# sunzeyucmu/VAE-based-Music--Deep-Generative-Models

Measured on AMD Instinct MI355X. Metric: audio-samples/sec/GPU VQ-VAE train step, 44.1kHz 65536-frame chunks @1/2/4/8 GPU, higher is better.
Workload: dtype bf16; 1 GPU; SMALL_VQ_VAE 3-level VQ-VAE train step (BASELINE config 2); model=VQVAE levels=3 latent=64 K=2048 down_depth=[3,2,2] width=32 depth=4 dil=3, global_batch=32, seq_len=65536, parallelism=dp1, graph=True

## Files before the change

include/vqa.h:

```cpp
#ifndef VQA_H
#define VQA_H

#include <stddef.h>
#include <stdint.h>

#ifdef __cplusplus
extern "C" {
#endif

typedef void* vqa_stream_t;

enum { VQA_OK = 0, VQA_E_INVALID_ARG = -1, VQA_E_UNSUPPORTED = -2, VQA_E_HIP = -3 };
enum { VQA_F32 = 0, VQA_BF16 = 1 };

enum {
  VQA_PRE_RELU = 1,
  VQA_ADD_RESIDUAL = 2,
  VQA_POST_MASK = 4,
  VQA_X_F32 = 8,
  VQA_Y_F32 = 16
};

const char* vqa_get_last_error(void);
const char* vqa_version(void);
// ... 62 lines not shown
  VQA_ROUTE_CO1 = 0, VQA_ROUTE_CONV32 = 1, VQA_ROUTE_GATHER_MFMA = 2, VQA_ROUTE_CI1 = 3, VQA_ROUTE_THIN_O = 4,
  VQA_ROUTE_THIN = 5, VQA_ROUTE_DIRECT = 6, VQA_ROUTE_WGRAD_MFMA = 7, VQA_ROUTE_WGRAD_THIN = 8,
  VQA_ROUTE_WGRAD_DIRECT = 9, VQA_ROUTE_TWO_CALL = 10
};
#define VQA_ROUTE_DETAIL 8
int vqa_conv1d_route(int op, int B, int T_in, int T_out, int C_in, int C_out, int K, int stride, int dilation,
                     int pad_left, int flags, int dtype, int* detail);

int vqa_resblock_supported(int C, int dilation, int dtype);
int vqa_resblock_fwd(const void* x, const float* wa, const float* ba, const float* wb, const float* bb, void* y,
                     void* h_out, int B, int T, int C, int dilation, int dtype, vqa_stream_t stream);
int vqa_resblock_bwd(const void* dy, const void* x, const float* wa, const float* ba, const float* wb, const float* bb,
                     void* dx, float* dwa, float* dba, float* dwb, float* dbb, int B, int T, int C, int dilation,
                     int dtype, void* workspace, size_t ws_bytes, vqa_partials_desc* desc, vqa_stream_t stream);
size_t vqa_resblock_bwd_workspace(int B, int T, int C, int dilation, int dtype);

int vqa_dtail_supported(int C, int Cu, int K_up, int stride_up, int K_out, int C_out, int dtype);
size_t vqa_dtail_workspace(int B, int T, int C, int Cu, int dtype);
int vqa_dtail_fwd(const void* h, const float* w_up, const float* b_up, const float* w_out, const float* b_out,
                  float* y, int B, int T, int C, int Cu, int dtype, void* workspace, size_t ws_bytes,
                  vqa_stream_t stream);
int vqa_dtail_bwd(const float* dy, const void* h, const float* w_up, const float* b_up, const float* w_out,
                  const float* b_out, void* dh, float* dw_up, float* db_up, float* dw_out, float* db_out, int B,
                  int T, int C, int Cu, int dtype, void* workspace, size_t ws_bytes, vqa_stream_t stream);

int vqa_vq_sqnorm(const float* E, float* e_sqnorm, int D, int K, vqa_stream_t stream);
int vqa_vq_argmin(const void* z, const float* E, const float* e_sqnorm, int64_t* idx, float* min_dist,
                  int64_t N, int D, int K, int dtype, vqa_stream_t stream);
int vqa_vq_argmin_split(const void* z, const void* E3, const float* e_sqnorm, int64_t* idx, float* min_dist,
                        int64_t N, int D, int K, vqa_stream_t stream);
// ... 145 lines not shown
```

vae-based-music--deep-generative-models_amd/csrc/vqa_resblock.hip:

```cpp
#include "vqa_launch.h"
#include "vqa_mfma.h"
#include <algorithm>
#include <type_traits>

namespace vqa {

constexpr int RC = 32;
constexpr int RTM = 128;
constexpr int RMAXD = 32;

struct ResArgs {
  const void* x;
  const void* dy;
  void* y;
  void* h;
  const float* wa;
  const float* ba;
  const float* wb;
  const float* bb;
  float* part_a;
  float* part_b;
  int B, T, d;
  int ntm, ntiles, tpw, textra;
  int nwg;
};

template <class T> constexpr int rs_stride() { return RC + lds_pad<T>(); }
constexpr int round16(int v) { return (v + 15) & ~15; }
constexpr int kVmcnt0 = 0x0F70;

#ifdef VQA_RS_STAMPS
constexpr int kRsStampWgs = 1024;
__device__ unsigned long long g_rs_stamps[kRsStampWgs * 4 * 8];
#define RS_STAMP(i)                                                                                      \
  do {                                                                                                   \
    if (stamp_on && lane == 0 && blockIdx.x < kRsStampWgs)                                               \
      g_rs_stamps[(blockIdx.x * 4 + wave) * 8 + (i)] = __builtin_amdgcn_s_memtime();                     \
  } while (0)
#else
// ... 198 lines not shown

struct RsCursor {
  int n, tm;
  __device__ __forceinline__ void set(int tile, int ntm) {
    n = tile / ntm;
    tm = tile - n * ntm;
  }
  __device__ __forceinline__ void next(int ntm) {
    if (++tm == ntm) {
      tm = 0;
      ++n;
    }
  }
};

template <class T> constexpr int rs_pv() { return sizeof(T) == 2 ? 4 : 8; }

template <class T> constexpr int rs_ncc() { return RC / Mfma<T>::KS; }

template <class T, bool KPERM>
__device__ __forceinline__ void load_wfrags(typename Mfma<T>::frag (&wf)[3][2][rs_ncc<T>()], const float* w) {
  const int lane = threadIdx.x & 63, m = lane & 15, kc = rs_kcol<T, KPERM>(lane);
#pragma unroll
  for (int k = 0; k < 3; ++k)
#pragma unroll
    for (int mt = 0; mt < 2; ++mt)
#pragma unroll
      for (int s = 0; s < rs_ncc<T>(); ++s) {
        const int o = 8 * rs_sig(m >> 2) + 4 * mt + (m & 3);
        if constexpr (sizeof(T) == 2) {
// ... 69 lines not shown
  if constexpr (sizeof(T) == 2) {
    __builtin_amdgcn_sched_group_barrier(0x100, NJ * 3 * NCC + (ALDS ? 6 * NCC : 0), 0);
    __builtin_amdgcn_sched_group_barrier(0x008, NJ * 6 * NCC, 0);
  }
}

__device__ __forceinline__ f32x4 bias4(const float* b, int o) { return f32x4{b[o], b[o + 1], b[o + 2], b[o + 3]}; }

constexpr bool kRsFwdKperm = false;

template <class T> constexpr int rs_fwd_waves() { return sizeof(T) == 2 ? 3 : 2; }

constexpr int rs_fwd_rt(int dt) { return dt > 0 ? 176 : RTM; }
constexpr int rs_bwd_rt(int dt) { return (dt > 0 && dt <= 9) ? 160 : RTM; }

template <class T, int DT, int RT = rs_fwd_rt(DT)>
__global__ __launch_bounds__(256) __attribute__((amdgpu_waves_per_eu(rs_fwd_waves<T>(), 8)))
void resblock_fwd_kernel(ResArgs a) {
  constexpr int XS = rs_stride<T>(), HR = RT + 16, NT = RT / 16, NJ = (NT + 3) / 4;
  extern __shared__ __attribute__((aligned(16))) char smem[];
  T* X = (T*)smem;
  const int d = DT > 0 ? DT : a.d, XR = HR + 2 * d;
  T* H = X + XR * XS;
  const int wave = __builtin_amdgcn_readfirstlane(threadIdx.x >> 6), lane = threadIdx.x & 63;
  const int tbeg = blockIdx.x * a.tpw + min((int)blockIdx.x, a.textra),
            tend = tbeg + a.tpw + ((int)blockIdx.x < a.textra);
  if (tbeg >= tend) return;
  typename Mfma<T>::frag wfa[3][2][rs_ncc<T>()], wfb[3][2][rs_ncc<T>()];
  if constexpr (sizeof(T) == 2 && DT > 0) {
    bf16* img = (bf16*)(X + (HR + 2 * DT) * XS);
    f32x4 va[3 * RC * RC / 4 / 256], vb[3 * RC * RC / 4 / 256];
    load_w4(va, a.wa);
    load_w4(vb, a.wb);
// ... 2 lines not shown
    __syncthreads();
    frags_from_img<kRsFwdKperm>(wfa, img);
    frags_from_img<kRsFwdKperm>(wfb, img + kImgRows * kImgP);
  } else {
    load_wfrags<T, kRsFwdKperm>(wfa, a.wa);
    load_wfrags<T, kRsFwdKperm>(wfb, a.wb);
  }
  const int pn = rs_pi(lane & 15), oc = rs_ocol(lane);
  f32x4 bav[2], bbv[2];
#pragma unroll
  for (int mt = 0; mt < 2; ++mt) {
    bav[mt] = a.ba ? bias4(a.ba, oc + 4 * mt) : f32x4{0.f, 0.f, 0.f, 0.f};
    bbv[mt] = a.bb ? bias4(a.bb, oc + 4 * mt) : f32x4{0.f, 0.f, 0.f, 0.f};
  }
  const unsigned ibytes = (unsigned)a.T * RC * (unsigned)sizeof(T);
  auto load_x = [&](Rows32Buf<T, rs_pv<T>()>& bx, const RsCursor& c) {
    bx.load(rs_rsrc((const T*)a.x + (size_t)c.n * a.T * RC, ibytes), c.tm * RT - 1 - d);
  };
  Rows32Buf<T, rs_pv<T>()> nx;
  nx.init(XR, (XR + HR) * XS);
  RsCursor cur, ldc;
  cur.set(tbeg, a.ntm);
  ldc = cur;
  load_x(nx, ldc);
  nx.template store<false>(X);
  if (tbeg + 1 < tend) {
    ldc.next(a.ntm);
    load_x(nx, ldc);
  }
  __syncthreads();
  for (int tile = tbeg; tile < tend; ++tile, cur.next(a.ntm)) {
    const int n = cur.n, t0 = cur.tm * RT;
#ifdef VQA_RS_STAMPS
    const bool stamp_on = tile == tbeg + 4;
#endif
    RS_STAMP(0);
    const bool interior = t0 - 1 >= 0 && t0 - 1 + HR <= a.T;
    int ry[NJ];
    Raw8<T> xres[NJ];
#pragma unroll
// ... 28 lines not shown
          for (int mt = 0; mt < 2; ++mt) {
            v[mt] = acc[j][mt];
#pragma unroll
            for (int q = 0; q < 4; ++q) v[mt][q] = live ? fmaxf(v[mt][q], 0.f) : 0.f;
          }
          st8(H + i * XS + oc, v[0], v[1]);
          if (a.h && i >= 1 && i <= RT)
            st8_buf<T>(rs_rsrc((T*)a.h + (size_t)n * a.T * RC, ibytes), (r * RC + oc) * (int)sizeof(T), v[0], v[1]);
        }
      }
    }
    RS_STAMP(1);
    __syncthreads();
    RS_STAMP(2);
    if (tile + 1 < tend) {
      nx.template store<false>(X);
      if (tile + 2 < tend) {
        ldc.next(a.ntm);
        load_x(nx, ldc);
      }
    }
    RS_STAMP(3);
    {
      const __amdgpu_buffer_rsrc_t yr = rs_rsrc((T*)a.y + (size_t)n * a.T * RC, ibytes);
      f32x4 acc[NJ][2];
      conv_multi<T, false, kRsFwdKperm, false, NJ>(acc, wb_frag, H, ry, 1, bbv[0], bbv[1]);
#pragma unroll
      for (int j = 0; j < NJ; ++j) {
        if (wave + 4 * j >= NT) continue;
        const int tl = ry[j] + pn;
        f32x4 x0, x1;
        xres[j].unpack(x0, x1);
        st8_buf<T>(yr, ((t0 + tl) * RC + oc) * (int)sizeof(T), x0 + acc[j][0], x1 + acc[j][1]);
      }
    }
    RS_STAMP(4);
    if (tile + 1 < tend) __syncthreads();
    RS_STAMP(5);
  }
}

template <class T, int DT, int RT = rs_bwd_rt(DT), int HALVES = 1>
__global__ __launch_bounds__(256 * HALVES) void resblock_bwd_kernel(ResArgs a) {
  typedef Mfma<T> M;
  constexpr int NW = 4;
  constexpr int XS = rs_stride<T>(), NT = RT / 16;
  constexpr int NA = (NT + 1) / 2, NA1 = NA < 3 ? NA : 3, NA2 = NA - NA1;
  static_assert(NA2 >= 1 && NA2 <= 3, "dx: two batches per team-W wave");
  constexpr int DM = DT > 0 ? DT : RMAXD, HRM = round16(RT + 2 * DM);
  constexpr int NHT = HRM / 16, NP1 = (NHT + 3) / 4, P1A = NP1 < 3 ? NP1 : 3, P1B = NP1 - P1A;
  constexpr int NDH = (NHT + 1) / 2, DH1 = NDH < 3 ? NDH : 3, DH2 = NDH - DH1 < 3 ? NDH - DH1 : 3,
                DH3 = NDH - DH1 - DH2;
  static_assert(P1B <= 3 && DH3 <= 3, "recomputed rows: at most 24 16-row tiles");
  constexpr int PVX = ((HRM + 2 * DM) * RC * (int)sizeof(T) / 16 + 64 * NW - 1) / (64 * NW);
  constexpr int PVY = ((HRM + 2) * RC * (int)sizeof(T) / 16 + 64 * NW - 1) / (64 * NW);
  extern __shared__ __attribute__((aligned(16))) char smem[];
  const int d = DT > 0 ? DT : a.d, HR = round16(RT + 2 * d), XR = HR + 2 * d, YR = HR + 2;
  const int wave_g = __builtin_amdgcn_readfirstlane(threadIdx.x >> 6);
// ... 27 lines not shown
    frags_from_img<true>(wt, img + (team == 0 ? 1 : 2) * kImgRows * kImgP);
  } else {
    load_wfrags<T, true>(wfa, a.wa);
    load_wfrags_t<T>(wt, team == 0 ? a.wa : a.wb);
  }
  const int pn = rs_pi(lane & 15), oc = rs_ocol(lane);
  f32x4 bav[2];
#pragma unroll
  for (int mt = 0; mt < 2; ++mt) bav[mt] = a.ba ? bias4(a.ba, oc + 4 * mt) : f32x4{0.f, 0.f, 0.f, 0.f};
  f32x4 gw[2][3], gb = {0.f, 0.f, 0.f, 0.f};
#pragma unroll
  for (int o = 0; o < 2; ++o)
#pragma unroll
    for (int k = 0; k < 3; ++k) gw[o][k] = f32x4{0.f, 0.f, 0.f, 0.f};
  const int nht = HR / 16;

  const unsigned ibytes = (unsigned)a.T * RC * (unsigned)sizeof(T);
  auto load_tile = [&](Rows32Buf<T, PVX>& bx, Rows32Buf<T, PVY>& by, const RsCursor& c) {
    const size_t o = (size_t)c.n * a.T * RC;
    bx.load(rs_rsrc((const T*)a.x + o, ibytes), c.tm * RT - 2 * d);
    by.load(rs_rsrc((const T*)a.dy + o, ibytes), c.tm * RT - d - 1);
  };
  Rows32Buf<T, PVX> nx;
  Rows32Buf<T, PVY> ny;
  nx.init(XR, (XR + YR + 2 * HR) * XS, (int)(threadIdx.x & 255));
  ny.init(YR, (YR + 2 * HR) * XS, (int)(threadIdx.x & 255));
  RsCursor cur, ldc;
  cur.set(min(tbeg + half, tend - 1), a.ntm);
  ldc = cur;
  if (tbeg + half < tend) {
    load_tile(nx, ny, ldc);
    nx.template store<true>(X);
    ny.template store<false>(Y);
// ... 1 lines not shown
  if (tbeg + half + HALVES < tend) {
    adv(ldc);
    load_tile(nx, ny, ldc);
  }
  __syncthreads();
  auto wt_frag = [&](int k, int mt, int sc) { return wt[k][mt][sc]; };
  for (int it = 0; it < niter; ++it, adv(cur)) {
    const int tile = tbeg + half + HALVES * it;
    const bool valid = HALVES == 1 || tile < tend;
    const int n = cur.n, t0 = cur.tm * RT;
    const bool interior = t0 - d >= 0 && t0 - d + HR <= a.T;
#ifdef VQA_RS_STAMPS
    const bool stamp_on = tile == tbeg + 4;
#endif
    RS_STAMP(0);
    auto h_batch = [&](auto nj, int j0) {
      constexpr int NJB = decltype(nj)::value;
      int rh[NJB];
#pragma unroll
      for (int j = 0; j < NJB; ++j) rh[j] = min(wave + 4 * (j0 + j), nht - 1) * 16;
      f32x4 acc[NJB][2];
      conv_multi<T, false, true, false, NJB>(acc, [&](int k, int mt, int sc) { return wfa[k][mt][sc]; }, X, rh, d,
                                             bav[0], bav[1]);
      if constexpr (sizeof(T) == 2) {
        auto store_h = [&](auto edge) {
#pragma unroll
          for (int j = 0; j < NJB; ++j) {
            if (wave + 4 * (j0 + j) >= nht) continue;
            const int i = rh[j] + pn;
            uint4 u = __builtin_bit_cast(uint4, relu_frag(__builtin_bit_cast(bf16x8, bf16_bits(acc[j][0], acc[j][1]))));
// ... 68 lines not shown
            for (int q = 0; q < 4; ++q) {
              dh[j][0][q] = hp[q] ? dh[j][0][q] : 0.f;
              dh[j][1][q] = hp[4 + q] ? dh[j][1][q] : 0.f;
            }
            st8(D + i * XS + oc, dh[j][0], dh[j][1]);
          }
        }
      };
      dh_batch(std::integral_constant<int, DH1>{}, 0);
      if constexpr (DH2 > 0) dh_batch(std::integral_constant<int, DH2>{}, DH1);
      if constexpr (DH3 > 0) dh_batch(std::integral_constant<int, DH3>{}, DH1 + DH2);
    }
    RS_STAMP(3);
    __syncthreads();
    RS_STAMP(4);
    __builtin_amdgcn_s_waitcnt(kVmcnt0);
    RS_STAMP(5);
    const __amdgpu_buffer_rsrc_t dxr = rs_rsrc((T*)a.y + (size_t)n * a.T * RC, ibytes);
    auto dx_batch = [&](auto nj, auto nt, auto frag) {
      constexpr int NJB = decltype(nj)::value;
      int rb[NJB];
      f32x4 acc[NJB][2];
#pragma unroll
      for (int j = 0; j < NJB; ++j) rb[j] = min(nt(j), NT - 1) * 16 + 2 * d;
      conv_multi<T, false, true, false, NJB>(acc, frag, D, rb, -d);
#pragma unroll
      for (int j = 0; j < NJB; ++j) {
        if (nt(j) >= NT) continue;
        const int tl = nt(j) * 16 + pn;
        bool xp[8];
        f32x4 y0, y1;
        pos8(X + (tl + 2 * d) * XS + oc, xp);
        ld8(Y + (tl + d + 1) * XS + oc, y0, y1);
#pragma unroll
        for (int q = 0; q < 4; ++q) {
          y0[q] += xp[q] ? acc[j][0][q] : 0.f;
          y1[q] += xp[4 + q] ? acc[j][1][q] : 0.f;
        }
        st8_buf<T>(dxr, ((t0 + tl) * RC + oc) * (int)sizeof(T), y0, y1);
      }
    };
    if (!valid) {
    } else if (team == 0) {
      dx_batch(std::integral_constant<int, NA1>{}, [&](int j) { return tw + 2 * j; }, wt_frag);
      dx_batch(std::integral_constant<int, NA2>{}, [&](int j) { return tw + 2 * (NA1 + j); }, wt_frag);
    } else {
#pragma unroll
      for (int kk = 0; kk < RT; kk += M::KS) {
        const typename M::frag b0 = rs_rows(D + (d + kk) * XS, XS);
        const typename M::frag b1 = rs_rows(D + (d + kk) * XS + 16, XS);
#pragma unroll
        for (int k = 0; k < 3; ++k) {
          const typename M::frag af = rs_rows(X + ((k + 1) * d + kk) * XS + tw * 16, XS);
          gw[0][k] = M::mma(af, b0, gw[0][k]);
          gw[1][k] = M::mma(af, b1, gw[1][k]);
        }
        gb = M::mma(M::ones(), tw ? b1 : b0, gb);
      }
    }
    RS_STAMP(6);
// ... 26 lines not shown
#pragma unroll
    for (int o = 0; o < 2; ++o)
#pragma unroll
      for (int k = 0; k < 3; ++k) gw[o][k] = gw[o][k] + *(const f32x4*)(xch + 4 * (3 * o + k));
    gb = gb + *(const f32x4*)(xch + 24);
  }
  float* pr = (team == 0 ? a.part_b : a.part_a) + (size_t)blockIdx.x * (3 * RC * RC + RC);
#pragma unroll
  for (int o = 0; o < 2; ++o)
#pragma unroll
    for (int k = 0; k < 3; ++k)
#pragma unroll
      for (int r = 0; r < 4; ++r)
        pr[(k * RC + tw * 16 + 4 * (lane >> 4) + r) * RC + o * 16 + (lane & 15)] = gw[o][k][r];
  if (lane < 16) pr[3 * RC * RC + tw * 16 + lane] = gb[0];
}

constexpr int kResPerCU = 2;
constexpr int kResMinTiles = 2;

static size_t fwd_lds(int d, int esz, int rt) {
  const int s = RC + 16 / esz, HR = rt + 16;
  return ((size_t)(HR + 2 * d) * s + (size_t)HR * s + s) * esz;
}
static size_t bwd_lds(int d, int esz, int rt) {
  const int s = RC + 16 / esz, HR = round16(rt + 2 * d);
  return ((size_t)(HR + 2 * d) * s + (size_t)(HR + 2) * s + (size_t)2 * HR * s + s) * esz;
}

template <class T> struct RsFwd {
// ... 106 lines not shown
  if (int rc = raise_dyn_lds(fn, lds_max, "resblock_bwd_kernel")) return rc;
  void* args[] = {&a};
  (void)hipLaunchKernel(fn, dim3(a.nwg), dim3(256), args, lds, s);
  VQA_LAUNCHED("resblock_bwd_kernel");
  const int nwg = a.nwg;
  const vqa_partials_desc da{a.part_a, dwa, dba, nwg, E, 3 * RC * RC, 0};
  const vqa_partials_desc dbd{a.part_b, dwb, dbb, nwg, E, 3 * RC * RC, 0};
  if (desc) {
    desc[0] = da;
    desc[1] = dbd;
    return VQA_OK;
  }
  const vqa_partials_desc both[2] = {da, dbd};
  return vqa_reduce_partials(both, 2, stream);
}
```

vae-based-music--deep-generative-models_amd/encdec.py:

```python
from __future__ import annotations

import torch

import vqa_lib as V
from resnet import DilatedResnet1D
from vqa_layers import Conv1D, Conv1DTranspose
from vqa_module import Layer


def print_dec_layer(decoder):
    for blk in decoder.blocks:
        print(f"-----{blk.prefix}-----")
        for res in blk.res:
            for rb in res.blocks:
                print(f"---------{rb.conv_a.name} (dilation {rb.dilation})---------")


class EncoderConvBlock(Layer):
    def __init__(self, output_dim, embed_width, embed_depth, dilation_factor=1, stride=2, down_depth=4, **kwargs):
        super().__init__(**kwargs)
        self.output_dim, self.embed_width, self.stride, self.down_depth = output_dim, embed_width, stride, down_depth
        self.kernel_size = stride * 2
        self.res = [DilatedResnet1D(embed_width, embed_depth, dilation_factor=dilation_factor) for _ in range(down_depth)]
        self._saved = None

    def _build(self, store, prefix, input_dim):
        self.prefix = prefix
        self.down = []
        cin = input_dim
        for i in range(self.down_depth):
            self.down.append(Conv1D(store, f"{prefix}/down{i}", cin, self.embed_width, self.kernel_size, self.stride))
            self.res[i].build(store, f"{prefix}/res{i}", self.embed_width, self.cdt)
            cin = self.embed_width
        self.proj = Conv1D(store, f"{prefix}/proj", self.embed_width, self.output_dim, 3)
        return self.output_dim

    def forward(self, x, save=False):
        ins = []
        for down, res in zip(self.down, self.res):
            ins.append(x)
            x = res.forward(down.forward(x, self.cdt), save)
        ins.append(x)
        self._saved = ins if save else None
        return self.proj.forward(x, self.cdt)

    def backward(self, dy, need_dx=True):
        ins = self._saved
        self._saved = None
        self.proj.backward_weight(ins[-1], dy, self.cdt)
        g = self.proj.backward_data(dy, ins[-1].shape[1], self.cdt)
        for i in reversed(range(self.down_depth)):
            g = self.res[i].backward(g)
            self.down[i].backward_weight(ins[i], g, self.cdt)
            if i > 0 or need_dx:
                g = self.down[i].backward_data(g, ins[i].shape[1], self.cdt, out_dtype=ins[i].dtype)
            else:
                g = None
        return g


class DecoderConvBlock(Layer):
    def __init__(self, output_dim, embed_width, embed_depth, dilation_factor=1, reverse_dilation=True,
                 dilation_cycle=None, stride=2, down_depth=4, **kwargs):
        super().__init__(**kwargs)
        self.output_dim, self.embed_width, self.stride, self.down_depth = output_dim, embed_width, stride, down_depth
        self.kernel_size = stride * 2
        self.res = [DilatedResnet1D(embed_width, embed_depth, dilation_factor=dilation_factor,
                                    reverse_dilation=reverse_dilation, dilation_cycle=dilation_cycle)
# ... 149 lines not shown
```

vae-based-music--deep-generative-models_amd/resnet.py:

```python
from __future__ import annotations

from typing import List, Optional

import torch

import vqa_lib as V
from vqa_layers import Conv1D
from vqa_module import Layer


class ResnetConv1DBlock(Layer):
    def __init__(self, input_dim, filters, dilation=1, **kwargs):
        super().__init__(**kwargs)
        self.input_dim, self.filters, self.dilation = input_dim, filters, dilation
        self._saved = None
        self._fused = None

    def _build(self, store, prefix, input_dim):
        assert input_dim == self.input_dim, f"{prefix}: input_dim {input_dim} != {self.input_dim}"
        self.conv_a = Conv1D(store, f"{prefix}/conv_a", self.input_dim, self.filters, 3, 1, self.dilation)
        self.conv_b = Conv1D(store, f"{prefix}/conv_b", self.filters, self.input_dim, 3, 1, 1)
        return self.input_dim

    def fused(self) -> bool:
        if self._fused is None:
            self._fused = (self.input_dim == self.filters and
                           V.resblock_supported(self.input_dim, self.dilation, V.dtype_code(self.cdt)))
        return self._fused

    def forward(self, x, save=False):
        if self.fused() and x.dtype == self.cdt:
            y = torch.empty_like(x)
            V.resblock_fwd(x, self.conv_a.w, self.conv_a.b, self.conv_b.w, self.conv_b.b, y, self.dilation)
            self._saved = (x, None) if save else None
            return y
        h = self.conv_a.forward(x, self.cdt, pre_relu=True)
        y = self.conv_b.forward(h, self.cdt, pre_relu=True, residual=x)
        self._saved = (x, h) if save else None
        return y

    def backward(self, dy):
        x, h = self._saved
        self._saved = None
        if h is None:
            st = self.store
            dx = torch.empty_like(x)
            V.resblock_bwd(dy, x, self.conv_a.w, self.conv_a.b, self.conv_b.w, self.conv_b.b, dx,
                           st.grad_view(f"{self.conv_a.name}/kernel"), st.grad_view(f"{self.conv_a.name}/bias"),
                           st.grad_view(f"{self.conv_b.name}/kernel"), st.grad_view(f"{self.conv_b.name}/bias"),
                           self.dilation, st.deferred)
            return dx
        dh = self.conv_b.backward_data_weight(dy, h, self.cdt, pre_relu=True)
        return self.conv_a.backward_data_weight(dh, x, self.cdt, pre_relu=True, residual=dy)


class DilatedResnet1D(Layer):
    def __init__(self, input_dim, depth, dilation_factor=1, reverse_dilation=False, dilation_cycle=None, **kwargs):
        super().__init__(**kwargs)
# ... 5 lines not shown
        self.dilations: List[int] = [_get_dilation(d) for d in range(depth)]
        if reverse_dilation:
            self.dilations = self.dilations[::-1]
        self.blocks = [ResnetConv1DBlock(input_dim, input_dim, dilation=d) for d in self.dilations]

    def _build(self, store, prefix, input_dim):
        for j, blk in enumerate(self.blocks):
            blk.build(store, f"{prefix}/rb{j}", input_dim, self.cdt)
        return input_dim

    def forward(self, x, save=False):
        for blk in self.blocks:
            x = blk.forward(x, save)
        return x

    def backward(self, dy):
        for blk in reversed(self.blocks):
            dy = blk.backward(dy)
        return dy
```

vae-based-music--deep-generative-models_amd/vqa_lib.py:

```python
from __future__ import annotations

import ctypes
import os
from typing import Optional

import torch

HERE = os.path.dirname(os.path.abspath(__file__))
LIB_PATH = os.environ.get("VQA_LIB_PATH") or os.path.join(HERE, "libvqa.so")

F32, BF16 = 0, 1
PRE_RELU, ADD_RESIDUAL, POST_MASK, X_F32, Y_F32 = 1, 2, 4, 8, 16

ABI_VERSION = 2

EXPORTED = [
    "vqa_get_last_error", "vqa_version", "vqa_abi_version", "vqa_same_pad_left", "vqa_same_out_len",
    "vqa_conv1d_fwd", "vqa_conv1d_bwd_data", "vqa_conv1d_bwd_weight", "vqa_conv1d_bwd_weight_workspace",
    "vqa_conv1d_transpose_fwd", "vqa_conv1d_transpose_bwd_data", "vqa_conv1d_transpose_bwd_weight",
    "vqa_conv1d_transpose_bwd_weight_workspace",
    "vqa_vq_sqnorm", "vqa_vq_argmin", "vqa_vq_quantize", "vqa_vq_quantize_workspace", "vqa_vq_backward",
    "vqa_vq_reset_rows", "vqa_vq_ema_apply", "vqa_vq_ema_apply_derived", "vqa_reset_perm_index",
    "vqa_mse_loss", "vqa_mse_loss_workspace", "vqa_adam_keras", "vqa_lr_schedule", "vqa_counter_add",
    "vqa_conv1d_bwd_weight_partials", "vqa_conv1d_transpose_bwd_weight_partials", "vqa_reduce_partials",
    "vqa_conv1d_bwd_data_weight", "vqa_conv1d_bwd_data_weight_workspace", "vqa_conv1d_route",
    "vqa_spectral_loss", "vqa_spectral_loss_workspace", "vqa_stft_magnitude",
    "vqa_vq_argmin_split", "vqa_vq_split_bf16x3",
    "vqa_resblock_supported", "vqa_resblock_fwd", "vqa_resblock_bwd", "vqa_resblock_bwd_workspace",
    "vqa_spectral_target_workspace", "vqa_spectral_target", "vqa_spectral_loss_target_workspace",
    "vqa_spectral_loss_target", "vqa_dtail_supported", "vqa_dtail_workspace", "vqa_dtail_fwd", "vqa_dtail_bwd",
    "vqa_step_metrics", "vqa_synthetic_batch",
    "vqa_embedding_fwd", "vqa_embedding_bwd", "vqa_embedding_bwd_workspace", "vqa_layernorm_fwd",
    "vqa_layernorm_bwd", "vqa_layernorm_bwd_workspace",
    "vqa_seqlin_fwd", "vqa_seqlin_prep", "vqa_seqlin_fwd_prepped", "vqa_seqlin_fwd_ln_prepped", "vqa_seqlin_wgrad_workspace", "vqa_seqlin_wgrad", "vqa_prior_embed_fwd", "vqa_colsum",
    "vqa_axpy", "vqa_dropout", "vqa_scale_f32", "vqa_tf_mix", "vqa_attn_fwd", "vqa_attn_bwd", "vqa_head_wt",
    "vqa_head_fwd", "vqa_head_bwd_workspace", "vqa_head_bwd", "vqa_rowsum_workspace", "vqa_rowsum", "vqa_prior_decode_cache_bytes",
    "vqa_prior_decode", "vqa_prior_decode_primed",
    "vqa_corpus_steps_per_epoch", "vqa_corpus_batch", "vqa_pcm_encode",
]


class VQAError(RuntimeError):
    pass
# ... 48 lines not shown
    "vqa_conv1d_bwd_weight_partials": (_I, [_P, _P, _P, _P] + _CONV + [_P, _S, _P, _P]),
    "vqa_conv1d_transpose_bwd_weight_partials": (_I, [_P, _P, _P, _P] + _CONVT + [_P, _S, _P, _P]),
    "vqa_reduce_partials": (_I, [_P, _I, _P]),
    "vqa_conv1d_bwd_data_weight": (_I, [_P, _P, _P, _P, _P, _P, _P] + _CONV + [_P, _S, _P, _P]),
    "vqa_conv1d_bwd_data_weight_workspace": (_S, _CONV),
    "vqa_conv1d_route": (_I, [_I] + _CONV + [_P]),
    "vqa_spectral_loss": (_I, [_P, _P, _P, _P, _P, _I, _I, _P, _P, _P, _I, _P, _S, _P]),
    "vqa_spectral_loss_workspace": (_S, [_I, _I, _P, _P, _P, _I, _I]),
    "vqa_stft_magnitude": (_I, [_P, _P, _I, _I, _I, _I, _I, _P]),
    "vqa_vq_argmin_split": (_I, [_P, _P, _P, _P, _P, _L, _I, _I, _P]),
    "vqa_vq_split_bf16x3": (_I, [_P, _P, _I, _I, _P]),
    "vqa_resblock_supported": (_I, [_I, _I, _I]),
    "vqa_resblock_fwd": (_I, [_P] * 7 + [_I] * 5 + [_P]),
    "vqa_resblock_bwd": (_I, [_P] * 11 + [_I] * 5 + [_P, _S, _P, _P]),
    "vqa_resblock_bwd_workspace": (_S, [_I] * 5),
    "vqa_dtail_supported": (_I, [_I] * 7),
    "vqa_dtail_workspace": (_S, [_I] * 5),
    "vqa_dtail_fwd": (_I, [_P] * 6 + [_I] * 5 + [_P, _S, _P]),
    "vqa_dtail_bwd": (_I, [_P] * 11 + [_I] * 5 + [_P, _S, _P]),
    "vqa_spectral_target_workspace": (_S, [_I, _I, _P, _P, _P, _I]),
    "vqa_spectral_target": (_I, [_P, _P, _S, _I, _I, _P, _P, _P, _I, _P]),
    "vqa_spectral_loss_target_workspace": (_S, [_I, _I, _P, _P, _P, _I, _I]),
    "vqa_spectral_loss_target": (_I, [_P, _P, _P, _P, _P, _I, _I, _P, _P, _P, _I, _P, _S, _P]),
    "vqa_seqlin_fwd": (_I, [_P, _L, _P, _P, _P, _L, _P, _L] + [_I] * 9 + [_P]),
    "vqa_seqlin_prep": (_I, [_P, _I, _I, _P]),
    "vqa_seqlin_fwd_prepped": (_I, [_P, _L, _P, _P, _P, _L, _P, _L] + [_I] * 8 + [_P]),
    "vqa_seqlin_fwd_ln_prepped": (_I, [_P, _L, _P, _P, ctypes.c_float, _P, _P, _P, _L, _P, _L] + [_I] * 7 + [_P]),
    "vqa_seqlin_wgrad_workspace": (_S, [_I] * 5),
    "vqa_seqlin_wgrad": (_I, [_P, _L, _P, _L, _P, _P] + [_I] * 6 + [_P, _S, _P, _P]),
    "vqa_prior_embed_fwd": (_I, [_P] * 6 + [_I] * 4 + [_F, _F, _U, _L, _P, _I, _P]),
# ... 208 lines not shown
                                  dtype_code(x.dtype), stream()), "vqa_resblock_fwd")


def resblock_bwd(dy, x, wa, ba, wb, bb, dx, dwa, dba, dwb, dbb, dilation, deferred=None):
    B, T, C = x.shape
    dt = dtype_code(x.dtype)
    ws = workspace(lib().vqa_resblock_bwd_workspace(B, T, C, dilation, dt), x.device)
    descs = (PartialsDesc * 2)() if deferred is not None else None
    _check(lib().vqa_resblock_bwd(ptr(dy), ptr(x), ptr(wa), ptr(ba), ptr(wb), ptr(bb), ptr(dx), ptr(dwa), ptr(dba),
                                  ptr(dwb), ptr(dbb), B, T, C, dilation, dt, ptr(ws), ws.numel(), descs, stream()),
           "vqa_resblock_bwd")
    if deferred is not None:
        deferred.add([descs[0], descs[1]], ws)


def conv1d_transpose_bwd_weight_deferred(x, dy, dw, db, B, T_in, T_out, C_in, C_out, K, stride, pad, flags, dtype,
                                         deferred):
    n = lib().vqa_conv1d_transpose_bwd_weight_workspace(B, T_in, T_out, C_in, C_out, K, stride, pad, flags, dtype)
    ws = workspace(n, x.device)
    d = PartialsDesc()
    _check(lib().vqa_conv1d_transpose_bwd_weight_partials(ptr(x), ptr(dy), ptr(dw), ptr(db), B, T_in, T_out, C_in,
                                                          C_out, K, stride, pad, flags, dtype, ptr(ws), ws.numel(),
                                                          ctypes.byref(d), stream()),
           "vqa_conv1d_transpose_bwd_weight_partials")
    deferred.add(d, ws)


def conv1d_transpose_fwd(x, w, b, residual, y, B, T_in, T_out, C_in, C_out, K, stride, pad, flags, dtype):
    _check(lib().vqa_conv1d_transpose_fwd(ptr(x), ptr(w), ptr(b), ptr(residual), ptr(y), B, T_in, T_out, C_in,
                                          C_out, K, stride, pad, flags, dtype, stream()), "vqa_conv1d_transpose_fwd")
# ... 450 lines not shown
```

Measured before the change: 328.7 million audio-samples/s.

## Fuse encoder input strided conv into first resblock forward and backward kernels

Adds fused kernels that compute the 1->32 channel, K=4 stride-2 input convolution of the waveform inside the first dilated resblock's tile staging, writing x as a side output. The backward kernel also accumulates the input-conv weight and bias gradients from the bf16 dx it produces, using per-workgroup partials. This removes a separate conv launch and a separate weight-gradient pass over the full-resolution activations. In exchange the resblock kernels carry more registers and extra scalar FMAs, and the fused path is on by default only when the first block's dx is not needed.

```diff
diff --git a/include/vqa.h b/include/vqa.h
--- a/include/vqa.h
+++ b/include/vqa.h
@@ -100,6 +100,16 @@
                      void* dx, float* dwa, float* dba, float* dwb, float* dbb, int B, int T, int C, int dilation,
                      int dtype, void* workspace, size_t ws_bytes, vqa_partials_desc* desc, vqa_stream_t stream);
 size_t vqa_resblock_bwd_workspace(int B, int T, int C, int dilation, int dtype);
+
+int vqa_resblock_in_supported(int C_in, int C_out, int K, int stride, int dilation, int dtype);
+int vqa_resblock_in_fwd(const float* wave, const float* w_in, const float* b_in, const float* wa, const float* ba,
+                        const float* wb, const float* bb, void* x, void* y, int B, int T_wave, int C_out, int K,
+                        int stride, int dilation, int dtype, vqa_stream_t stream);
+int vqa_resblock_in_bwd(const void* dy, const void* x, const float* wave, const float* wa, const float* ba,
+                        const float* wb, const float* bb, void* dx, float* dwa, float* dba, float* dwb, float* dbb,
+                        float* dw_in, float* db_in, int B, int T_wave, int C_out, int K, int stride, int dilation,
+                        int dtype, void* workspace, size_t ws_bytes, vqa_partials_desc* desc, vqa_stream_t stream);
+size_t vqa_resblock_in_bwd_workspace(int B, int T_wave, int C_out, int K, int stride, int dilation, int dtype);
 
 int vqa_dtail_supported(int C, int Cu, int K_up, int stride_up, int K_out, int C_out, int dtype);
 size_t vqa_dtail_workspace(int B, int T, int C, int Cu, int dtype);
diff --git a/vae-based-music--deep-generative-models_amd/csrc/vqa_resblock.hip b/vae-based-music--deep-generative-models_amd/csrc/vqa_resblock.hip
--- a/vae-based-music--deep-generative-models_amd/csrc/vqa_resblock.hip
+++ b/vae-based-music--deep-generative-models_amd/csrc/vqa_resblock.hip
@@ -23,6 +23,11 @@
   int B, T, d;
   int ntm, ntiles, tpw, textra;
   int nwg;
+  const float* wave;
+  const float* win;
+  const float* bin;
+  float* part_in;
+  int Tw, pin;
 };
 
 template <class T> constexpr int rs_stride() { return RC + lds_pad<T>(); }
@@ -251,6 +256,67 @@
   }
 };
 
+constexpr int kInK = 4, kInS = 2, kInE = kInK * RC + RC;
+
+struct RowsIn {
+  static constexpr int PV = 4;
+  float s[PV][kInK];
+  int rr[PV], loff[PV];
+  int lt0, ln;
+  __device__ __forceinline__ void init(int nrows, int trash) {
+    constexpr int XS = RC + 8;
+#pragma unroll
+    for (int i = 0; i < PV; ++i) {
+      const int e = threadIdx.x + i * 256, G = e >> 3;
+      const int r = 8 * (G >> 2) + (G & 3) + 4 * ((e >> 2) & 1), q = e & 3;
+      const bool in = r < nrows;
+      rr[i] = in ? r : -(1 << 24);
+      loff[i] = in ? r * XS + q * 8 : trash;
+    }
+  }
+  __device__ __forceinline__ void load(const ResArgs& a, const RsCursor& c, int row0) {
+    lt0 = row0;
+    ln = c.n;
+    const __amdgpu_buffer_rsrc_t r = rs_rsrc(a.wave + (size_t)c.n * a.Tw, (unsigned)a.Tw * 4u);
+#pragma unroll
+    for (int i = 0; i < PV; ++i) {
+      const int t = row0 + rr[i], i0 = kInS * t - a.pin;
+      const bool live = (unsigned)t < (unsigned)a.T;
+#pragma unroll
+      for (int k = 0; k < kInK; ++k) {
+        const bool ok = live && (unsigned)(i0 + k) < (unsigned)a.Tw;
+        s[i][k] = __builtin_bit_cast(float, __builtin_amdgcn_raw_buffer_load_b32(r, ok ? (i0 + k) * 4 : kRsOOB, 0, 0));
+      }
+    }
+  }
+  __device__ __forceinline__ void store(const ResArgs& a, bf16* X, const float (&w)[kInK][8], const float (&b)[8],
+                                        int own0, int rt) const {
+    const __amdgpu_buffer_rsrc_t xr =
+        rs_rsrc((bf16*)a.x + (size_t)ln * a.T * RC, (unsigned)a.T * RC * (unsigned)sizeof(bf16));
+    const int q8 = 8 * (threadIdx.x & 3);
+#pragma unroll
+    for (int i = 0; i < PV; ++i) {
+      const int t = lt0 + rr[i];
+      const bool live = (unsigned)t < (unsigned)a.T;
+      float acc[8];
+#pragma unroll
+      for (int j = 0; j < 8; ++j) acc[j] = 0.f;
+#pragma unroll
+      for (int k = 0; k < kInK; ++k)
+#pragma unroll
+        for (int j = 0; j < 8; ++j) acc[j] += s[i][k] * w[k][j];
+#pragma unroll
+      for (int j = 0; j < 8; ++j) acc[j] = acc[j] + b[j];
+      uint4 u = uint4{pk_bf16(acc[0], acc[1]), pk_bf16(acc[2], acc[3]), pk_bf16(acc[4], acc[5]), pk_bf16(acc[6], acc[7])};
+      if (!live) u = uint4{0u, 0u, 0u, 0u};
+      *(uint4*)(X + loff[i]) = u;
+      const bool own = live && rr[i] >= own0 && rr[i] < own0 + rt;
+      __builtin_amdgcn_raw_buffer_store_b128(__builtin_bit_cast(v4u32, u), xr,
+                                             own ? (t * RC + q8) * (int)sizeof(bf16) : kRsOOB, 0, 0);
+    }
+  }
+};
+
 template <class T> constexpr int rs_pv() { return sizeof(T) == 2 ? 4 : 8; }
 
 template <class T> constexpr int rs_ncc() { return RC / Mfma<T>::KS; }
@@ -350,9 +416,9 @@
 constexpr int rs_fwd_rt(int dt) { return dt > 0 ? 176 : RTM; }
 constexpr int rs_bwd_rt(int dt) { return (dt > 0 && dt <= 9) ? 160 : RTM; }
 
-template <class T, int DT, int RT = rs_fwd_rt(DT)>
-__global__ __launch_bounds__(256) __attribute__((amdgpu_waves_per_eu(rs_fwd_waves<T>(), 8)))
-void resblock_fwd_kernel(ResArgs a) {
+template <class T, int DT, int RT, bool IN>
+__device__ __forceinline__ void resblock_fwd_body(const ResArgs& a) {
+  static_assert(!IN || (sizeof(T) == 2 && DT == 1), "the fused input conv: bf16, dilation 1");
   constexpr int XS = rs_stride<T>(), HR = RT + 16, NT = RT / 16, NJ = (NT + 3) / 4;
   extern __shared__ __attribute__((aligned(16))) char smem[];
   T* X = (T*)smem;
@@ -385,16 +451,32 @@
     bbv[mt] = a.bb ? bias4(a.bb, oc + 4 * mt) : f32x4{0.f, 0.f, 0.f, 0.f};
   }
   const unsigned ibytes = (unsigned)a.T * RC * (unsigned)sizeof(T);
-  auto load_x = [&](Rows32Buf<T, rs_pv<T>()>& bx, const RsCursor& c) {
-    bx.load(rs_rsrc((const T*)a.x + (size_t)c.n * a.T * RC, ibytes), c.tm * RT - 1 - d);
+  typedef std::conditional_t<IN, RowsIn, Rows32Buf<T, rs_pv<T>()>> Stager;
+  float win[IN ? kInK : 1][8], bin[8];
+  if constexpr (IN) {
+    const int q8 = 8 * (threadIdx.x & 3);
+#pragma unroll
+    for (int k = 0; k < kInK; ++k)
+#pragma unroll
+      for (int j = 0; j < 8; ++j) win[k][j] = a.win[k * RC + q8 + j];
+#pragma unroll
+    for (int j = 0; j < 8; ++j) bin[j] = a.bin ? a.bin[q8 + j] : 0.f;
+  }
+  auto load_x = [&](Stager& bx, const RsCursor& c) {
+    if constexpr (IN) bx.load(a, c, c.tm * RT - 1 - d);
+    else bx.load(rs_rsrc((const T*)a.x + (size_t)c.n * a.T * RC, ibytes), c.tm * RT - 1 - d);
   };
-  Rows32Buf<T, rs_pv<T>()> nx;
+  auto store_x = [&](const Stager& bx) {
+    if constexpr (IN) bx.store(a, X, win, bin, 1 + d, RT);
+    else bx.template store<false>(X);
+  };
+  Stager nx;
   nx.init(XR, (XR + HR) * XS);
   RsCursor cur, ldc;
   cur.set(tbeg, a.ntm);
   ldc = cur;
   load_x(nx, ldc);
-  nx.template store<false>(X);
+  store_x(nx);
   if (tbeg + 1 < tend) {
     ldc.next(a.ntm);
     load_x(nx, ldc);
@@ -453,7 +535,7 @@
     __syncthreads();
     RS_STAMP(2);
     if (tile + 1 < tend) {
-      nx.template store<false>(X);
+      store_x(nx);
       if (tile + 2 < tend) {
         ldc.next(a.ntm);
         load_x(nx, ldc);
@@ -479,8 +561,21 @@
   }
 }
 
-template <class T, int DT, int RT = rs_bwd_rt(DT), int HALVES = 1>
-__global__ __launch_bounds__(256 * HALVES) void resblock_bwd_kernel(ResArgs a) {
+template <class T, int DT, int RT = rs_fwd_rt(DT)>
+__global__ __launch_bounds__(256) __attribute__((amdgpu_waves_per_eu(rs_fwd_waves<T>(), 8)))
+void resblock_fwd_kernel(ResArgs a) {
+  resblock_fwd_body<T, DT, RT, false>(a);
+}
+
+constexpr int kResInFwdPerCU = 2;
+__global__ __launch_bounds__(256) __attribute__((amdgpu_waves_per_eu(kResInFwdPerCU, 8)))
+void resblock_in_fwd_kernel(ResArgs a) {
+  resblock_fwd_body<bf16, 1, rs_fwd_rt(1), true>(a);
+}
+
+template <class T, int DT, int RT, int HALVES, bool IN>
+__device__ __forceinline__ void resblock_bwd_body(const ResArgs& a) {
+  static_assert(!IN || (sizeof(T) == 2 && DT == 1 && HALVES == 1), "the fused input conv: bf16, dilation 1");
   typedef Mfma<T> M;
   constexpr int NW = 4;
   constexpr int XS = rs_stride<T>(), NT = RT / 16;
@@ -538,9 +633,18 @@
 #pragma unroll
     for (int k = 0; k < 3; ++k) gw[o][k] = f32x4{0.f, 0.f, 0.f, 0.f};
   const int nht = HR / 16;
+  float gin[IN ? kInK : 1][8], gbin[8];
+  if constexpr (IN) {
+#pragma unroll
+    for (int j = 0; j < 8; ++j) {
+      gbin[j] = 0.f;
+#pragma unroll
+      for (int k = 0; k < kInK; ++k) gin[k][j] = 0.f;
+    }
+  }
 
   const unsigned ibytes = (unsigned)a.T * RC * (unsigned)sizeof(T);
-  auto load_tile = [&](Rows32Buf<T, PVX>& bx, Rows32Buf<T, PVY>& by, const RsCursor& c) {
+  auto load_tile =[&](Rows32Buf<T, PVX>& bx, Rows32Buf<T, PVY>& by, const RsCursor& c) {
     const size_t o = (size_t)c.n * a.T * RC;
     bx.load(rs_rsrc((const T*)a.x + o, ibytes), c.tm * RT - 2 * d);
     by.load(rs_rsrc((const T*)a.dy + o, ibytes), c.tm * RT - d - 1);
@@ -572,6 +676,27 @@
     const bool stamp_on = tile == tbeg + 4;
 #endif
     RS_STAMP(0);
+    float sw[IN ? NA : 1][kInK];
+    auto load_sw = [&] {
+      if constexpr (IN) {
+      if (team == 0) {
+        const __amdgpu_buffer_rsrc_t wr = rs_rsrc(a.wave + (size_t)n * a.Tw, (unsigned)a.Tw * 4u);
+#pragma unroll
+        for (int j = 0; j < NA; ++j) {
+          const int nt = tw + 2 * j, t = t0 + nt * 16 + pn, i0 = kInS * t - a.pin;
+          const bool live = nt < NT && t < a.T;
+#pragma unroll
+          for (int k = 0; k < kInK; ++k) {
+            const bool ok = live && (unsigned)(i0 + k) < (unsigned)a.Tw;
+            sw[j][k] =
+                __builtin_bit_cast(float, __builtin_amdgcn_raw_buffer_load_b32(wr, ok ? (i0 + k) * 4 : kRsOOB, 0, 0));
+          }
+        }
+      }
+      }
+    };
+    constexpr bool kSwEarly = RT != 128;
+    if constexpr (kSwEarly) load_sw();
     auto h_batch = [&](auto nj, int j0) {
       constexpr int NJB = decltype(nj)::value;
       int rh[NJB];
@@ -670,11 +795,12 @@
     RS_STAMP(3);
     __syncthreads();
     RS_STAMP(4);
+    if constexpr (!kSwEarly) load_sw();
     __builtin_amdgcn_s_waitcnt(kVmcnt0);
     RS_STAMP(5);
     const __amdgpu_buffer_rsrc_t dxr = rs_rsrc((T*)a.y + (size_t)n * a.T * RC, ibytes);
-    auto dx_batch = [&](auto nj, auto nt, auto frag) {
-      constexpr int NJB = decltype(nj)::value;
+    auto dx_batch = [&](auto nj, auto jb, auto nt, auto frag) {
+      constexpr int NJB = decltype(nj)::value, J0 = decltype(jb)::value;
       int rb[NJB];
       f32x4 acc[NJB][2];
 #pragma unroll
@@ -693,13 +819,29 @@
           y0[q] += xp[q] ? acc[j][0][q] : 0.f;
           y1[q] += xp[4 + q] ? acc[j][1][q] : 0.f;
         }
-        st8_buf<T>(dxr, ((t0 + tl) * RC + oc) * (int)sizeof(T), y0, y1);
+        if constexpr (IN) {
+          const uint4 u = bf16_bits(y0, y1);
+          __builtin_amdgcn_raw_buffer_store_b128(__builtin_bit_cast(v4u32, u), dxr,
+                                                 ((t0 + tl) * RC + oc) * (int)sizeof(T), 0, 0);
+          const unsigned uw[4] = {u.x, u.y, u.z, u.w};
+#pragma unroll
+          for (int c = 0; c < 8; ++c) {
+            const float g = __uint_as_float((c & 1) ? (uw[c >> 1] & 0xFFFF0000u) : (uw[c >> 1] << 16));
+            gbin[c] += g;
+#pragma unroll
+            for (int k = 0; k < kInK; ++k) gin[k][c] = __builtin_fmaf(sw[J0 + j][k], g, gin[k][c]);
+          }
+        } else {
+          st8_buf<T>(dxr, ((t0 + tl) * RC + oc) * (int)sizeof(T), y0, y1);
+        }
       }
     };
     if (!valid) {
     } else if (team == 0) {
-      dx_batch(std::integral_constant<int, NA1>{}, [&](int j) { return tw + 2 * j; }, wt_frag);
-      dx_batch(std::integral_constant<int, NA2>{}, [&](int j) { return tw + 2 * (NA1 + j); }, wt_frag);
+      dx_batch(std::integral_constant<int, NA1>{}, std::integral_constant<int, 0>{}, [&](int j) { return tw + 2 * j; },
+               wt_frag);
+      dx_batch(std::integral_constant<int, NA2>{}, std::integral_constant<int, NA1>{},
+               [&](int j) { return tw + 2 * (NA1 + j); }, wt_frag);
     } else {
 #pragma unroll
       for (int kk = 0; kk < RT; kk += M::KS) {
@@ -756,6 +898,38 @@
       for (int r = 0; r < 4; ++r)
         pr[(k * RC + tw * 16 + 4 * (lane >> 4) + r) * RC + o * 16 + (lane & 15)] = gw[o][k][r];
   if (lane < 16) pr[3 * RC * RC + tw * 16 + lane] = gb[0];
+  if constexpr (IN) {
+    __syncthreads();
+    float* red = (float*)smem;
+    if (team == 0) {
+#pragma unroll
+      for (int c = 0; c < 8; ++c) {
+        gbin[c] = xl::row_sum(gbin[c]);
+#pragma unroll
+        for (int k = 0; k < kInK; ++k) gin[k][c] = xl::row_sum(gin[k][c]);
+      }
+      if ((lane & 15) == 0) {
+#pragma unroll
+        for (int c = 0; c < 8; ++c) {
+          red[tw * kInE + kInK * RC + oc + c] = gbin[c];
+#pragma unroll
+          for (int k = 0; k < kInK; ++k) red[tw * kInE + k * RC + oc + c] = gin[k][c];
+        }
+      }
+    }
+    __syncthreads();
+    if (threadIdx.x < kInE) a.part_in[(size_t)blockIdx.x * kInE + threadIdx.x] = red[threadIdx.x] + red[kInE + threadIdx.x];
+  }
+}
+
+template <class T, int DT, int RT = rs_bwd_rt(DT), int HALVES = 1>
+__global__ __launch_bounds__(256 * HALVES) void resblock_bwd_kernel(ResArgs a) {
+  resblock_bwd_body<T, DT, RT, HALVES, false>(a);
+}
+
+template <int RT>
+__global__ __launch_bounds__(256) void resblock_in_bwd_kernel(ResArgs a) {
+  resblock_bwd_body<bf16, 1, RT, 1, true>(a);
 }
 
 constexpr int kResPerCU = 2;
@@ -892,3 +1066,86 @@
   const vqa_partials_desc both[2] = {da, dbd};
   return vqa_reduce_partials(both, 2, stream);
 }
+
+extern "C" int vqa_resblock_in_supported(int C_in, int C_out, int K, int stride, int dilation, int dtype) {
+  return C_in == 1 && C_out == RC && K == kInK && stride == kInS && dilation == 1 && dtype == VQA_BF16 &&
+         vqa_resblock_supported(RC, 1, VQA_BF16);
+}
+
+static int resblock_in_check(const char* what, int B, int T_wave, int C_out, int K, int stride, int dilation, int dtype,
+                             int* T) {
+  VQA_ARG(B > 0 && T_wave > 0, "%s: bad sizes B=%d T_wave=%d", what, B, T_wave);
+  VQA_REQUIRE(vqa_resblock_in_supported(1, C_out, K, stride, dilation, dtype), VQA_E_UNSUPPORTED,
+              "%s: unsupported C_out=%d K=%d stride=%d dilation=%d dtype=%d", what, C_out, K, stride, dilation, dtype);
+  *T = vqa_same_out_len(T_wave, kInS);
+  VQA_ARG((long long)*T * RC * 4 < (1ll << 30), "%s: item too long for 32-bit buffer offsets (T_wave=%d)", what, T_wave);
+  return VQA_OK;
+}
+
+extern "C" int vqa_resblock_in_fwd(const float* wave, const float* w_in, const float* b_in, const float* wa,
+                                   const float* ba, const float* wb, const float* bb, void* x, void* y, int B,
+                                   int T_wave, int C_out, int K, int stride, int dilation, int dtype,
+                                   vqa_stream_t stream) {
+  VQA_ARG(wave && w_in && wa && wb && x && y, "resblock_in_fwd: null tensor pointer");
+  int T = 0;
+  if (int rc = resblock_in_check("resblock_in_fwd", B, T_wave, C_out, K, stride, dilation, dtype, &T)) return rc;
+  ResArgs a{x, nullptr, y, nullptr, wa, ba, wb, bb, nullptr, nullptr, B, T, 1, 0, 0, 0, 0, 0};
+  a.wave = wave;
+  a.win = w_in;
+  a.bin = b_in;
+  a.Tw = T_wave;
+  a.pin = vqa_same_pad_left(T_wave, kInK, kInS, 1);
+  plan(a, kResInFwdPerCU, rs_fwd_rt(1));
+  const size_t lds = fwd_lds(1, 2, rs_fwd_rt(1));
+  const void* fn = (const void*)resblock_in_fwd_kernel;
+  if (int rc = raise_dyn_lds(fn, lds, "resblock_in_fwd_kernel")) return rc;
+  void* args[] = {&a};
+  (void)hipLaunchKernel(fn, dim3(a.nwg), dim3(256), args, lds, (hipStream_t)stream);
+  VQA_LAUNCHED("resblock_in_fwd_kernel");
+  return VQA_OK;
+}
+
+extern "C" size_t vqa_resblock_in_bwd_workspace(int B, int T_wave, int C_out, int K, int stride, int dilation,
+                                                int dtype) {
+  if (B < 1 || T_wave < 1 || !vqa_resblock_in_supported(1, C_out, K, stride, dilation, dtype)) return 0;
+  return vqa_resblock_bwd_workspace(B, vqa_same_out_len(T_wave, kInS), RC, 1, dtype) +
+         (size_t)cu_count() * kResPerCU * kInE * sizeof(float);
+}
+
+extern "C" int vqa_resblock_in_bwd(const void* dy, const void* x, const float* wave, const float* wa, const float* ba,
+                                   const float* wb, const float* bb, void* dx, float* dwa, float* dba, float* dwb,
+                                   float* dbb, float* dw_in, float* db_in, int B, int T_wave, int C_out, int K,
+                                   int stride, int dilation, int dtype, void* workspace, size_t ws_bytes,
+                                   vqa_partials_desc* desc, vqa_stream_t stream) {
+  (void)bb;
+  VQA_ARG(dy && x && wave && wa && wb && dx && dwa && dwb && dw_in, "resblock_in_bwd: null tensor pointer");
+  int T = 0;
+  if (int rc = resblock_in_check("resblock_in_bwd", B, T_wave, C_out, K, stride, dilation, dtype, &T)) return rc;
+  const size_t need = vqa_resblock_in_bwd_workspace(B, T_wave, C_out, K, stride, dilation, dtype);
+  VQA_ARG(workspace && ws_bytes >= need, "resblock_in_bwd: workspace %zu < %zu bytes", ws_bytes, need);
+  const int E = 3 * RC * RC + RC;
+  ResArgs a{x, dy, dx, nullptr, wa, ba, wb, nullptr, (float*)workspace, nullptr, B, T, 1, 0, 0, 0, 0, 0};
+  const int rt = bwd_rt_for(1, T);
+  plan(a, kResPerCU, rt, kResMinTiles);
+  a.part_b = a.part_a + (size_t)a.nwg * E;
+  a.part_in = a.part_b + (size_t)a.nwg * E;
+  a.wave = wave;
+  a.Tw = T_wave;
+  a.pin = vqa_same_pad_left(T_wave, kInK, kInS, 1);
+  const size_t lds = bwd_lds(1, 2, rt);
+  const void* fn = rt == 128 ? (const void*)resblock_in_bwd_kernel<128> : (const void*)resblock_in_bwd_kernel<rs_bwd_rt(1)>;
+  if (int rc = raise_dyn_lds(fn, std::max(bwd_lds(1, 2, 128), bwd_lds(1, 2, rs_bwd_rt(1))), "resblock_in_bwd_kernel"))
+    return rc;
+  void* args[] = {&a};
+  (void)hipLaunchKernel(fn, dim3(a.nwg), dim3(256), args, lds, (hipStream_t)stream);
+  VQA_LAUNCHED("resblock_in_bwd_kernel");
+  const int nwg = a.nwg;
+  const vqa_partials_desc d3[3] = {{a.part_a, dwa, dba, nwg, E, 3 * RC * RC, 0},
+                                   {a.part_b, dwb, dbb, nwg, E, 3 * RC * RC, 0},
+                                   {a.part_in, dw_in, db_in, nwg, kInE, kInK * RC, 0}};
+  if (desc) {
+    for (int i = 0; i < 3; ++i) desc[i] = d3[i];
+    return VQA_OK;
+  }
+  return vqa_reduce_partials(d3, 3, stream);
+}
diff --git a/vae-based-music--deep-generative-models_amd/encdec.py b/vae-based-music--deep-generative-models_amd/encdec.py
--- a/vae-based-music--deep-generative-models_amd/encdec.py
+++ b/vae-based-music--deep-generative-models_amd/encdec.py
@@ -1,4 +1,6 @@
 from __future__ import annotations
+
+import os
 
 import torch
 
@@ -17,12 +19,15 @@
 
 
 class EncoderConvBlock(Layer):
-    def __init__(self, output_dim, embed_width, embed_depth, dilation_factor=1, stride=2, down_depth=4, **kwargs):
+    def __init__(self, output_dim, embed_width, embed_depth, dilation_factor=1, stride=2, down_depth=4, fuse_in=None,
+                 **kwargs):
         super().__init__(**kwargs)
         self.output_dim, self.embed_width, self.stride, self.down_depth = output_dim, embed_width, stride, down_depth
         self.kernel_size = stride * 2
         self.res = [DilatedResnet1D(embed_width, embed_depth, dilation_factor=dilation_factor) for _ in range(down_depth)]
         self._saved = None
+        self.fuse_in = os.environ.get("VQA_FUSE_IN", "1") != "0" if fuse_in is None else bool(fuse_in)
+        self._fused_in = False
 
     def _build(self, store, prefix, input_dim):
         self.prefix = prefix
@@ -37,9 +42,14 @@
 
     def forward(self, x, save=False):
         ins = []
-        for down, res in zip(self.down, self.res):
+        self._fused_in = False
+        for i, (down, res) in enumerate(zip(self.down, self.res)):
             ins.append(x)
-            x = res.forward(down.forward(x, self.cdt), save)
+            if i == 0 and save and self.fuse_in and res.blocks and res.blocks[0].fused_in(down, x):
+                x = res.forward_in(down, x, save)
+                self._fused_in = True
+            else:
+                x = res.forward(down.forward(x, self.cdt), save)
         ins.append(x)
         self._saved = ins if save else None
         return self.proj.forward(x, self.cdt)
@@ -50,8 +60,12 @@
         self.proj.backward_weight(ins[-1], dy, self.cdt)
         g = self.proj.backward_data(dy, ins[-1].shape[1], self.cdt)
         for i in reversed(range(self.down_depth)):
+            fused_in = i == 0 and self._fused_in and not need_dx
+            if i == 0 and self._fused_in and need_dx:
+                self.res[0].blocks[0].drop_in()
             g = self.res[i].backward(g)
-            self.down[i].backward_weight(ins[i], g, self.cdt)
+            if not fused_in:
+                self.down[i].backward_weight(ins[i], g, self.cdt)
             if i > 0 or need_dx:
                 g = self.down[i].backward_data(g, ins[i].shape[1], self.cdt, out_dtype=ins[i].dtype)
             else:
diff --git a/vae-based-music--deep-generative-models_amd/resnet.py b/vae-based-music--deep-generative-models_amd/resnet.py
--- a/vae-based-music--deep-generative-models_amd/resnet.py
+++ b/vae-based-music--deep-generative-models_amd/resnet.py
@@ -15,6 +15,7 @@
         self.input_dim, self.filters, self.dilation = input_dim, filters, dilation
         self._saved = None
         self._fused = None
+        self._in = None
 
     def _build(self, store, prefix, input_dim):
         assert input_dim == self.input_dim, f"{prefix}: input_dim {input_dim} != {self.input_dim}"
@@ -39,9 +40,37 @@
         self._saved = (x, h) if save else None
         return y
 
+    def fused_in(self, conv, wave) -> bool:
+        return (self.fused() and wave.dtype == torch.float32 and conv.d == 1 and
+                V.resblock_in_supported(conv.cin, conv.cout, conv.K, conv.s, self.dilation, V.dtype_code(self.cdt)))
+
+    def forward_in(self, conv, wave, save=False):
+        B, Tw, _ = wave.shape
+        x = torch.empty((B, conv.out_len(Tw), conv.cout), dtype=self.cdt, device=wave.device)
+        y = torch.empty_like(x)
+        V.resblock_in_fwd(wave, conv.w, conv.b, self.conv_a.w, self.conv_a.b, self.conv_b.w, self.conv_b.b, x, y,
+                          conv.s, self.dilation)
+        self._saved = (x, None) if save else None
+        self._in = (conv, wave) if save else None
+        return y
+
+    def drop_in(self):
+        self._in = None
+
     def backward(self, dy):
         x, h = self._saved
         self._saved = None
+        fin, self._in = self._in, None
+        if fin is not None:
+            conv, wave = fin
+            st = self.store
+            dx = torch.empty_like(x)
+            V.resblock_in_bwd(dy, x, wave, self.conv_a.w, self.conv_a.b, self.conv_b.w, self.conv_b.b, dx,
+                              st.grad_view(f"{self.conv_a.name}/kernel"), st.grad_view(f"{self.conv_a.name}/bias"),
+                              st.grad_view(f"{self.conv_b.name}/kernel"), st.grad_view(f"{self.conv_b.name}/bias"),
+                              st.grad_view(f"{conv.name}/kernel"), st.grad_view(f"{conv.name}/bias"), conv.s,
+                              self.dilation, st.deferred)
+            return dx
         if h is None:
             st = self.store
             dx = torch.empty_like(x)
@@ -77,6 +106,12 @@
             x = blk.forward(x, save)
         return x
 
+    def forward_in(self, conv, wave, save=False):
+        x = self.blocks[0].forward_in(conv, wave, save)
+        for blk in self.blocks[1:]:
+            x = blk.forward(x, save)
+        return x
+
     def backward(self, dy):
         for blk in reversed(self.blocks):
             dy = blk.backward(dy)
diff --git a/vae-based-music--deep-generative-models_amd/vqa_lib.py b/vae-based-music--deep-generative-models_amd/vqa_lib.py
--- a/vae-based-music--deep-generative-models_amd/vqa_lib.py
+++ b/vae-based-music--deep-generative-models_amd/vqa_lib.py
@@ -27,6 +27,7 @@
     "vqa_spectral_loss", "vqa_spectral_loss_workspace", "vqa_stft_magnitude",
     "vqa_vq_argmin_split", "vqa_vq_split_bf16x3",
     "vqa_resblock_supported", "vqa_resblock_fwd", "vqa_resblock_bwd", "vqa_resblock_bwd_workspace",
+    "vqa_resblock_in_supported", "vqa_resblock_in_fwd", "vqa_resblock_in_bwd", "vqa_resblock_in_bwd_workspace",
     "vqa_spectral_target_workspace", "vqa_spectral_target", "vqa_spectral_loss_target_workspace",
     "vqa_spectral_loss_target", "vqa_dtail_supported", "vqa_dtail_workspace", "vqa_dtail_fwd", "vqa_dtail_bwd",
     "vqa_step_metrics", "vqa_synthetic_batch",
@@ -105,6 +106,10 @@
     "vqa_resblock_fwd": (_I, [_P] * 7 + [_I] * 5 + [_P]),
     "vqa_resblock_bwd": (_I, [_P] * 11 + [_I] * 5 + [_P, _S, _P, _P]),
     "vqa_resblock_bwd_workspace": (_S, [_I] * 5),
+    "vqa_resblock_in_supported": (_I, [_I] * 6),
+    "vqa_resblock_in_fwd": (_I, [_P] * 9 + [_I] * 7 + [_P]),
+    "vqa_resblock_in_bwd": (_I, [_P] * 14 + [_I] * 7 + [_P, _S, _P, _P]),
+    "vqa_resblock_in_bwd_workspace": (_S, [_I] * 7),
     "vqa_dtail_supported": (_I, [_I] * 7),
     "vqa_dtail_workspace": (_S, [_I] * 5),
     "vqa_dtail_fwd": (_I, [_P] * 6 + [_I] * 5 + [_P, _S, _P]),
@@ -343,6 +348,33 @@
         deferred.add([descs[0], descs[1]], ws)
 
 
+def resblock_in_supported(C_in, C_out, K, stride, dilation, dtype) -> bool:
+    return bool(lib().vqa_resblock_in_supported(C_in, C_out, K, stride, dilation, dtype))
+
+
+def resblock_in_fwd(wave, w_in, b_in, wa, ba, wb, bb, x, y, stride=2, dilation=1):
+    B, Tw = wave.shape[0], wave.shape[1]
+    K, _, C = w_in.shape
+    _check(lib().vqa_resblock_in_fwd(ptr(wave), ptr(w_in), ptr(b_in), ptr(wa), ptr(ba), ptr(wb), ptr(bb), ptr(x),
+                                     ptr(y), B, Tw, C, K, stride, dilation, dtype_code(x.dtype), stream()),
+           "vqa_resblock_in_fwd")
+
+
+def resblock_in_bwd(dy, x, wave, wa, ba, wb, bb, dx, dwa, dba, dwb, dbb, dw_in, db_in, stride=2, dilation=1,
+                    deferred=None):
+    B, Tw = wave.shape[0], wave.shape[1]
+    K, _, C = dw_in.shape
+    dt = dtype_code(x.dtype)
+    ws = workspace(lib().vqa_resblock_in_bwd_workspace(B, Tw, C, K, stride, dilation, dt), x.device)
+    descs = (PartialsDesc * 3)() if deferred is not None else None
+    _check(lib().vqa_resblock_in_bwd(ptr(dy), ptr(x), ptr(wave), ptr(wa), ptr(ba), ptr(wb), ptr(bb), ptr(dx),
+                                     ptr(dwa), ptr(dba), ptr(dwb), ptr(dbb), ptr(dw_in), ptr(db_in), B, Tw, C, K,
+                                     stride, dilation, dt, ptr(ws), ws.numel(), descs, stream()),
+           "vqa_resblock_in_bwd")
+    if deferred is not None:
+        deferred.add([descs[0], descs[1], descs[2]], ws)
+
+
 def conv1d_transpose_bwd_weight_deferred(x, dy, dw, db, B, T_in, T_out, C_in, C_out, K, stride, pad, flags, dtype,
                                          deferred):
     n = lib().vqa_conv1d_transpose_bwd_weight_workspace(B, T_in, T_out, C_in, C_out, K, stride, pad, flags, dtype)
```

Measured after the change: 328.3 million audio-samples/s, median of 2. No clear change (-0.1%).
